# EvolEcolGroup/tidypopgen

Measured on AMD Instinct MI355X. Metric: SNP-genotypes/s (N x M) for IBS+KING+GRM+Fst+PCA; max |delta| vs CPU ref (cpu_baseline.parity), higher is better.
Workload: dtype fp4-e2m1 operands (exact integers, f32 accumulate) for the cross-products, the PCA Gram and the grouped counts, int8 (int32 accumulate) for the loadings, f64 for statistics

## Files before the change

include/tpg.h:

```cpp
#ifndef TPG_H
#define TPG_H

#include <stddef.h>
#include <stdint.h>

#ifdef __cplusplus
extern "C" {
#endif

#define TPG_OK 0
#define TPG_EINVAL 1
#define TPG_EHIP 2
#define TPG_EUNSUPPORTED 3
#define TPG_ENUMERIC 4

typedef struct tpg_ctx tpg_ctx;
typedef struct tpg_fbm tpg_fbm;
typedef struct tpg_view tpg_view;
typedef struct tpg_pairwise tpg_pairwise;
typedef struct tpg_comm tpg_comm;
typedef struct tpg_multi tpg_multi;

const char* tpg_last_error(void);
const char* tpg_version(void);
// ... 391 lines not shown
  size_t bytes_up;
  size_t bytes_down;
  size_t budget_bytes;
  size_t planned_bytes;
  size_t state_bytes;
  size_t peak_device_bytes;
  double seconds;
  double seconds_first_sweep;
} tpg_stream_report;

int tpg_stream_run(tpg_ctx* ctx, tpg_stream* s, const tpg_stream_job* job, tpg_stream_report* report);
int tpg_multi_stream_run(tpg_multi* mg, tpg_stream* s, const tpg_stream_job* job, tpg_stream_report* report);

typedef struct tpg_stream_qc_job {
  size_t struct_size;
  const int32_t* rowInd1;
  int64_t n;
  const int32_t* colInd1;
  int64_t m;
  const double* code256;
  const int32_t* groupIds0;
  int ngroups;
  int midp;
  int32_t* loci_counts;
  double* hwe_p;
  int32_t* grouped_counts;
  double* grouped_hwe_p;
  int32_t* indiv_counts;
} tpg_stream_qc_job;
int tpg_stream_qc(tpg_ctx* ctx, tpg_stream* s, const tpg_stream_qc_job* job, tpg_stream_report* report);

int tpg_pca_center_scale(tpg_ctx* ctx, const tpg_view* v, double* center, double* scale);
int tpg_pca_gram(tpg_ctx* ctx, const tpg_view* v, const double* center, const double* scale, double* K);
int tpg_pca_gram_add(tpg_ctx* ctx, const tpg_view* v, const double* center, const double* scale, double* K);
int tpg_pca_partial_svd(tpg_ctx* ctx, const tpg_view* v, int k, double* d, double* u, double* vload,
                        double* center, double* scale, double* square_frobenius);
int tpg_pca_random_svd(tpg_ctx* ctx, const tpg_view* v, int k, double tol, double* d, double* u, double* vload,
                       double* center, double* scale, double* square_frobenius);
int tpg_sym_eig_topk(tpg_ctx* ctx, const double* K, int64_t n, int k, double* lambda, double* U);
int tpg_pca_loadings(tpg_ctx* ctx, const tpg_view* v, const double* center, const double* scale,
                     const double* U, const double* d, int k, double* vload);
int tpg_fbm256_prod_and_rowSumsSq(tpg_ctx* ctx, const tpg_view* v, const double* center,
                                  const double* scale, const double* V, int K, double* XV, double* rss);
int tpg_square_frobenius(tpg_ctx* ctx, const tpg_view* v, const double* center, const double* scale,
                         double* out);
int tpg_fbm256_valid_prod(tpg_ctx* ctx, const tpg_view* v, const double* Tab, int K, double* out);

#define TPG_PCA_OP_TOL_FLOOR 1e-8
int tpg_pca_zt_prod(tpg_ctx* ctx, const tpg_view* v, const double* center, const double* scale, const double* Q, int b,
                    double* W);
int tpg_pca_z_prod(tpg_ctx* ctx, const tpg_view* v, const double* center, const double* scale, const double* W, int b,
                   double* Y);
int tpg_pca_random_svd_op(tpg_ctx* ctx, const tpg_view* v, int k, double tol, double* d, double* u, double* vload,
                          double* center, double* scale, double* square_frobenius, int* n_apply);
size_t tpg_pca_op_scratch_bytes(int64_t n, int64_t m, int k);
int tpg_pca_gram_route_fits(tpg_ctx* ctx, int64_t n, int k, int* fits);

#define TPG_PCADAPT_MAX_K 64
#define TPG_SELECT_TILE 1024
int64_t tpg_select_tile(void);
int tpg_col_median_mad(tpg_ctx* ctx, const double* X, int64_t rows, int ncols, int64_t ld, double* med, double* mad,
                       int64_t* n_finite);
int tpg_pcadapt_zscores(tpg_ctx* ctx, const tpg_view* v, const double* U, int K, double* z, int64_t* n_valid);
int tpg_robust_dist_ogk(tpg_ctx* ctx, const double* Z, int64_t m, int K, double* dist, double* center, double* cov,
                        double* basis, int64_t* n_valid);
int tpg_pchisq_log10_upper(tpg_ctx* ctx, const double* x, int64_t count, int df, double* out);
// ... 84 lines not shown
```

tidypopgen_amd/_lib.py:

```python
from __future__ import annotations

import ctypes as C
import os

_HERE = os.path.dirname(os.path.abspath(__file__))
LIB_PATH = os.environ.get("TPG_LIB_PATH") or os.path.join(_HERE, "libtpg_hip.so")


class TpgError(RuntimeError):
    def __init__(self, code: int, msg: str):
        super().__init__(f"[tpg error {code}] {msg}")
        self.code = code


def build(force: bool = False) -> str:
    import subprocess

    csrc = os.path.join(_HERE, "csrc")
    cmd = ["make", "-C", csrc, "-j8", "-s"]
    if force:
        cmd.append("-B")
    subprocess.check_call(cmd)
    return LIB_PATH

# ... 206 lines not shown
    "tpg_comm_rank": (ci, [vp]),
    "tpg_comm_size": (ci, [vp]),
    "tpg_shard_loci": (ci, [i64, ci, ci, vp, vp]),
    "tpg_comm_allreduce_f64": (ci, [vp, vp, vp, i64]),
    "tpg_pairwise_buffer_bytes_sharded": (sz, [i64, ci]),
    "tpg_pairwise_create_sharded": (ci, [vp, vp, i64, vp]),
    "tpg_pairwise_reduce": (ci, [vp, vp, vp]),
    "tpg_pairwise_reduce_begin": (ci, [vp, vp, vp]),
    "tpg_pairwise_reduce_end": (ci, [vp, vp, vp]),
    "tpg_pairwise_band": (ci, [vp, vp, vp]),
    "tpg_pairwise_band_of": (ci, [i64, ci, ci, vp, vp]),
    "tpg_pairwise_epilogues_sharded": (ci, [vp, vp, vp, ci, i64, vp, vp, vp, vp]),
    "tpg_pca_partial_svd_sharded": (ci, [vp, vp, vp, ci, vp, vp, vp, vp, vp, vp]),
    "tpg_multi_create": (ci, [ci, vp, vp]),
    "tpg_multi_destroy": (None, [vp]),
    "tpg_multi_ndev": (ci, [vp]),
    "tpg_multi_ctx": (vp, [vp, ci]),
    "tpg_multi_comm": (vp, [vp, ci]),
    "tpg_multi_pairwise": (ci, [vp, vp, i64, i64, vp, i64, vp, i64, ci, vp, vp, vp, vp]),
    "tpg_multi_grouped_alt_freq": (ci, [vp, vp, i64, i64, vp, i64, vp, i64, vp, vp, ci, vp, ci, vp]),
    "tpg_multi_pop_fst": (ci, [vp, vp, i64, i64, vp, i64, vp, i64, vp, vp, ci, vp, ci, vp, ci, ci, ci, vp, vp, vp]),
    "tpg_multi_pca_partial_svd": (ci, [vp, vp, i64, i64, vp, i64, vp, i64, vp, ci, vp, vp, vp, vp, vp, vp]),
    "tpg_stream_open_host": (ci, [vp, vp, i64, i64, sz, vp]),
    "tpg_stream_open_bk": (ci, [vp, cstr, i64, i64, sz, vp]),
    "tpg_stream_open_bed": (ci, [vp, cstr, i64, i64, sz, vp]),
    "tpg_stream_open_bed_host": (ci, [vp, vp, i64, i64, sz, vp]),
    "tpg_stream_open_synth": (ci, [vp, u64, i64, i64, ci, u32, ci, sz, vp]),
    "tpg_stream_close": (None, [vp]),
    "tpg_stream_run": (ci, [vp, vp, P(StreamJob), P(StreamReport)]),
    "tpg_multi_stream_run": (ci, [vp, vp, P(StreamJob), P(StreamReport)]),
    "tpg_stream_qc": (ci, [vp, vp, P(StreamQcJob), P(StreamReport)]),
    "tpg_pca_center_scale": (ci, [vp, vp, vp, vp]),
    "tpg_pca_gram": (ci, [vp, vp, vp, vp, vp]),
    "tpg_pca_gram_add": (ci, [vp, vp, vp, vp, vp]),
    "tpg_pca_partial_svd": (ci, [vp, vp, ci, vp, vp, vp, vp, vp, vp]),
    "tpg_pca_random_svd": (ci, [vp, vp, ci, f64, vp, vp, vp, vp, vp, vp]),
    "tpg_sym_eig_topk": (ci, [vp, vp, i64, ci, vp, vp]),
    "tpg_pca_loadings": (ci, [vp, vp, vp, vp, vp, vp, ci, vp]),
    "tpg_fbm256_prod_and_rowSumsSq": (ci, [vp, vp, vp, vp, vp, ci, vp, vp]),
    "tpg_square_frobenius": (ci, [vp, vp, vp, vp, vp]),
    "tpg_fbm256_valid_prod": (ci, [vp, vp, vp, ci, vp]),
    "tpg_pca_zt_prod": (ci, [vp, vp, vp, vp, vp, ci, vp]),
    "tpg_pca_z_prod": (ci, [vp, vp, vp, vp, vp, ci, vp]),
    "tpg_pca_random_svd_op": (ci, [vp, vp, ci, f64, vp, vp, vp, vp, vp, vp, vp]),
    "tpg_pca_op_scratch_bytes": (sz, [i64, i64, ci]),
    "tpg_pca_gram_route_fits": (ci, [vp, i64, ci, vp]),
    "tpg_select_tile": (i64, []),
    "tpg_col_median_mad": (ci, [vp, vp, i64, ci, i64, vp, vp, vp]),
    "tpg_pcadapt_zscores": (ci, [vp, vp, vp, ci, vp, vp]),
    "tpg_robust_dist_ogk": (ci, [vp, vp, i64, ci, vp, vp, vp, vp, vp]),
    "tpg_pchisq_log10_upper": (ci, [vp, vp, i64, ci, vp]),
    "tpg_qchisq_median": (ci, [ci, vp]),
    "tpg_pcadapt": (ci, [vp, vp, vp, ci, vp, vp, vp, vp, vp, vp]),
    "tpg_view_select_loci": (ci, [vp, vp, vp, i64, vp]),
    "tpg_qnorm_upper": (ci, [f64, vp]),
    "tpg_rollmean_weights": (ci, [ci, vp]),
    "tpg_rollmean_segments": (ci, [vp, vp, i64, vp, i64, ci, vp]),
    "tpg_medcouple": (ci, [vp, vp, i64, vp]),
    "tpg_tukey_mc_up": (ci, [vp, vp, i64, f64, vp]),
    "tpg_pca_auto_svd": (ci, [vp, vp, vp, vp, ci, f64, ci, f64, i64, ci, vp]),
    "tpg_autosvd_count": (i64, [vp]),
    "tpg_autosvd_iters": (ci, [vp]),
    "tpg_autosvd_converged": (ci, [vp]),
    "tpg_autosvd_fetch": (ci, [vp, vp, vp, vp, vp, vp, vp, vp]),
    "tpg_autosvd_history": (ci, [vp, ci, vp, vp, vp]),
    "tpg_autosvd_outliers": (ci, [vp, ci, vp, vp]),
# ... 40 lines not shown
```

tidypopgen_amd/api.py:

```python
from __future__ import annotations

import ctypes as C
import math
from typing import Optional

import numpy as np

from . import _lib
from ._lib import check, lib

CODE_012 = np.full(256, np.nan)
CODE_012[:3] = [0.0, 1.0, 2.0]
CODE_IMPUTE_PRED = np.full(256, np.nan)
CODE_IMPUTE_PRED[:3] = [0.0, 1.0, 2.0]
CODE_IMPUTE_PRED[4:7] = [0.0, 1.0, 2.0]

FST_METHODS = {"Hudson": 0, "Nei87": 1, "WC84": 2}
IMPUTE_METHODS = {"mode": 1, "mean0": 2, "random": 3}


def _impute_method(method) -> int:
    if method not in IMPUTE_METHODS:
        raise ValueError(f"impute method must be one of {sorted(IMPUTE_METHODS)}, not {method!r}")
    return IMPUTE_METHODS[method]
# ... 2271 lines not shown
    check(lib.tpg_pairwise_fst_loop(ctx.h, FST_METHODS[method], _ptr(pairs_c), P, m,
                                    G, _ptr(n), *[_ptr(x) for x in mats], int(by_locus),
                                    int(return_num_dem), _ptr(tot), _ptr(a), _ptr(b)))
    return _fst_result(tot, a, b, by_locus or return_num_dem, return_num_dem)


def pairwise_fst_hudson_loop(pairwise_combn, n, freq_alt, freq_ref, by_locus=False, return_num_dem=False, ctx=None):
    return _fst_loop("Hudson", pairwise_combn, n, freq_alt, freq_ref, None, by_locus, return_num_dem, ctx)


def pairwise_fst_wc84_loop(pairwise_combn, n, freq_alt, het_obs, by_locus=False, return_num_dem=False, ctx=None):
    return _fst_loop("WC84", pairwise_combn, n, freq_alt, None, het_obs, by_locus, return_num_dem, ctx)


def pairwise_fst_nei87_loop(pairwise_combn, n, het_obs, freq_alt, freq_ref, by_locus=False, return_num_dem=False,
                            ctx=None):
    return _fst_loop("Nei87", pairwise_combn, n, freq_alt, freq_ref, het_obs, by_locus, return_num_dem, ctx)



def pca_center_scale(v: View):
    center, scale = np.zeros(v.m), np.zeros(v.m)
    check(lib.tpg_pca_center_scale(v.ctx.h, v.h, _ptr(center), _ptr(scale)))
    return center, scale


def pca_gram(v: View, center, scale) -> np.ndarray:
    K = np.zeros((v.n, v.n), order="F")
    center, scale = _f64(center), _f64(scale)
    check(lib.tpg_pca_gram(v.ctx.h, v.h, _ptr(center), _ptr(scale), _ptr(K)))
    return K


def sym_eig_topk(K, k: int, ctx: Optional[Context] = None):
    ctx = ctx or default_context()
    K = np.asfortranarray(K, dtype=float)
    n = K.shape[0]
    lam, U = np.zeros(k), np.zeros((n, k), order="F")
    check(lib.tpg_sym_eig_topk(ctx.h, _ptr(K), n, k, _ptr(lam), _ptr(U)))
    return lam, U


def pca_loadings(v: View, center, scale, U, d) -> np.ndarray:
    center, scale, d = _f64(center), _f64(scale), _f64(d)
    U = np.asfortranarray(U, dtype=float)
    k = U.shape[1]
    out = np.zeros((v.m, k), order="F")
    check(lib.tpg_pca_loadings(v.ctx.h, v.h, _ptr(center), _ptr(scale), _ptr(U), _ptr(d), k, _ptr(out)))
    return out


def _pca_view(X: FBM, ind_row, ind_col, code256, impute, impute_seed) -> View:
    if impute is None:
        return View(X, ind_row, ind_col, code256=code256)
    return View(X, ind_row, ind_col, code256=CODE_012).impute(impute, impute_seed)


def gt_pca_partialSVD(X: FBM, ind_row=None, ind_col=None, k: int = 10, total_var: bool = True,
                      code256=CODE_IMPUTE_PRED, impute: Optional[str] = None, impute_seed: int = 0) -> dict:
    v = _pca_view(X, ind_row, ind_col, code256, impute, impute_seed)
    d = np.zeros(k)
    u = np.zeros((v.n, k), order="F")
    vl = np.zeros((v.m, k), order="F")
    center, scale = np.zeros(v.m), np.zeros(v.m)
    fro = C.c_double()
    check(lib.tpg_pca_partial_svd(v.ctx.h, v.h, k, _ptr(d), _ptr(u), _ptr(vl), _ptr(center), _ptr(scale),
# ... 817 lines not shown
```

tidypopgen_amd/csrc/gramcls.hip:

```cpp
#include <math.h>
#include <string.h>

#include <algorithm>
#include <vector>

#include <hipcub/hipcub.hpp>

#include "common.h"
#include "devfrag.h"
#include "host/host_bits2.h"

constexpr int GA = 2, GB = 2, GP = GA * GB;
#define GCLS_SLAB (GP * 16 * 64)
#define GCLS_MAX_RUN 65536

__global__ void tpg_gcls_keys_kernel(const double* __restrict__ w, int64_t m, unsigned long long* __restrict__ key,
                                     uint32_t* __restrict__ idx) {
  for (int64_t j = blockIdx.x * (int64_t)blockDim.x + threadIdx.x; j < m; j += (int64_t)gridDim.x * blockDim.x) {
    const unsigned long long b = (unsigned long long)__double_as_longlong(w[j]);
    key[j] = (b + 16ull) & ~31ull;
    idx[j] = (uint32_t)j;
  }
}

// ... 37 lines not shown
__global__ void tpg_gcls_block_table_kernel(const unsigned long long* __restrict__ ukeys, const uint32_t* __restrict__ blk_start,
                                            const uint32_t* __restrict__ nblk, int nr, int64_t nblocks,
                                            unsigned long long* __restrict__ wblk) {
  for (int64_t b = blockIdx.x * (int64_t)blockDim.x + threadIdx.x; b < nblocks; b += (int64_t)gridDim.x * blockDim.x) {
    const int r = tpg_gcls_find_run(blk_start, nr, (uint32_t)b);
    const uint32_t o = (uint32_t)b - blk_start[r];
    const unsigned long long fl = (o + 1 == nblk[r] || (o % GCLS_MAX_RUN) == GCLS_MAX_RUN - 1) ? 1ull : 0ull;
    wblk[b] = ukeys[r] | fl;
  }
}

#define GCLS_GQ 6
#define GCLS_GMAX 64
#define GCLS_GRUN 16384
__global__ void tpg_gcls_block_table2_kernel(const unsigned long long* __restrict__ ukeys, const uint32_t* __restrict__ blk_start,
                                             const uint32_t* __restrict__ nblk, int nr, int64_t nblocks, int gmax, int gq,
                                             ulonglong2* __restrict__ wblk) {
  if (blockIdx.x == 0 && threadIdx.x < 4) wblk[nblocks + threadIdx.x] = make_ulonglong2(ukeys[nr - 1], 0ull);
  for (int64_t b = blockIdx.x * (int64_t)blockDim.x + threadIdx.x; b < nblocks; b += (int64_t)gridDim.x * blockDim.x) {
    const int r = tpg_gcls_find_run(blk_start, nr, (uint32_t)b);
    const uint32_t o = (uint32_t)b - blk_start[r];
    const bool class_end = o + 1 == nblk[r];
    bool full = (o % GCLS_GRUN) == GCLS_GRUN - 1;
    if (class_end)
      full = full || r == nr - 1 || (ukeys[r] >> (52 - gq)) != (ukeys[r + 1] >> (52 - gq)) ||
             (r % gmax) == gmax - 1 || blk_start[r] / GCLS_GRUN != (blk_start[r] + nblk[r]) / GCLS_GRUN;
    ulonglong2 e;
    e.x = ukeys[r] | (full ? 2ull : class_end ? 1ull : 0ull);
    e.y = 0;
    if (class_end && !full)
      e.y = (unsigned long long)__float_as_uint(
          (float)(__longlong_as_double((long long)ukeys[r]) - __longlong_as_double((long long)ukeys[r + 1])));
    wblk[b] = e;
  }
}

struct GclsSrc {
  const uint4* base;
  int sh;
  int64_t sa;
  int msk;
  int64_t sb, sq, sh1;
};

#define GSH_ROW 68
#define GSH_HS 140
#define GSH_WORDS (4 * 2 * GSH_HS)
template <bool CEN, int QW>
__global__ __launch_bounds__(256) void tpg_gcls_gather_kernel(GclsSrc S, int64_t Q,
                                                               const int32_t* __restrict__ src, int64_t nblocks,
                                                               int64_t rs2, uint4* __restrict__ T2g) {
  __shared__ __attribute__((aligned(16))) uint32_t shm[4][GSH_WORDS];
  const int lane = threadIdx.x & 63, wv = threadIdx.x >> 6;
  uint32_t* sh = shm[wv];
  const int g = lane & 3, x = lane >> 2, t_s = x & 3, t_hs = (x >> 2) & 1, t_hb = x >> 3;
  const uint4* rd_src = (const uint4*)(sh + x * GSH_ROW + 16 * g);
  uint32_t* wr_dst = sh + t_s * (2 * GSH_HS) + t_hs * GSH_HS + (g >> 1) * 4 + 2 * t_hb + (g & 1);
  const int r = lane & 31, ho = lane >> 5;
  const uint4* rd_dst = (const uint4*)(sh + (r >> 4) * GSH_HS + (r & 15) * 8 + ho * 4);
  const uint32_t uQ = (uint32_t)((Q + QW - 1) / QW), ntask = uQ * (uint32_t)rs2, step = gridDim.x * 4u;
  auto load_j = [&](uint32_t task, int32_t (&j)[2]) {
    j[0] = j[1] = -1;
    if (task < ntask) {
      const int64_t bp = task / uQ;
#pragma unroll
      for (int hb = 0; hb < 2; hb++)
// ... 419 lines not shown
    __builtin_amdgcn_fence(__ATOMIC_ACQUIRE, "workgroup");
    const int a = lane & 31, h = lane >> 5;
#pragma unroll 4
    for (int it = 0; it < 16; it++) {
      const int c = 2 * it + h;
      const int i1 = 32 * ti + a, k1 = 32 * tk + c;
      if (i1 < n && k1 < n) K[i1 + (int64_t)k1 * n] = tile[p][a][c];
      const int i2 = 32 * ti + c, k2 = 32 * tk + a;
      if (i2 < n && k2 < n) K[k2 + (int64_t)i2 * n] = tile[p][c][a];
    }
    __builtin_amdgcn_wave_barrier();
  }
}

static bool gcls_fold64(int64_t nruns, int64_t nblocks) {
  if (tpg_env_set("TPG_GRAM_FOLD64")) return tpg_env_int("TPG_GRAM_FOLD64", 0) != 0;
  return (double)nruns < 0.15 * (double)nblocks;
}

static double gcls_cost_classes(int64_t nunits, int64_t nruns, int64_t nblocks, int nwaves, int* bestS) {
  double best = -1;
  const bool f64 = gcls_fold64(nruns, nblocks);
  const double t_class = f64 ? 0.136 : GCLS2_T_CLASS, t_block = f64 ? 0.079 : GCLS2_T_BLOCK;
  for (int S = 2; S <= 32; S += 2) {
    if (nblocks / S < 4 && S > 2) break;
    const int64_t rounds = ceil_div(nunits * S, (int64_t)nwaves);
    const double per = ((double)nruns / S + 1.0) * GP * t_class + (double)ceil_div(nblocks, (int64_t)S) * GP * t_block + 6.0;
    const double cost = (double)rounds * per + (double)S * (double)nunits * 8.5e-3;
    if (best < 0 || cost < best * 0.995) { best = cost; *bestS = S; }
  }
  return best;
}

static int gram_classes_core(tpg_ctx* ctx, int64_t n, int64_t Q, int64_t m, const GclsSrc& src, const double* d_w, double* d_what,
                             double* d_K, bool force, bool* done, bool centred_ok) {
  *done = false;
  if (m >= (1ll << 31) - 64 || (tpg_env_set("TPG_GRAM_DIGITS") && !force)) return TPG_OK;
  DevArena B;
  unsigned long long *d_key = nullptr, *d_key2 = nullptr, *d_ukeys = nullptr;
  uint32_t *d_idx = nullptr, *d_idx2 = nullptr, *d_counts = nullptr, *d_cnt = nullptr, *d_nblk = nullptr, *d_estart = nullptr,
           *d_bstart = nullptr;
  int* d_nruns = nullptr;
  long long* d_totals = nullptr;
  void* d_tmp = nullptr;
  TPG_TRY(B.get(&d_key, (size_t)m)); TPG_TRY(B.get(&d_key2, (size_t)m)); TPG_TRY(B.get(&d_ukeys, (size_t)m));
  TPG_TRY(B.get(&d_idx, (size_t)m)); TPG_TRY(B.get(&d_idx2, (size_t)m)); TPG_TRY(B.get(&d_counts, (size_t)m));
  TPG_TRY(B.get(&d_cnt, (size_t)m)); TPG_TRY(B.get(&d_nblk, (size_t)m)); TPG_TRY(B.get(&d_estart, (size_t)m));
  TPG_TRY(B.get(&d_bstart, (size_t)m)); TPG_TRY(B.get(&d_nruns, 1)); TPG_TRY(B.get(&d_totals, 2));
  size_t t_sort = 0, t_rle = 0, t_scan = 0;
  TPG_HIP(hipcub::DeviceRadixSort::SortPairs(nullptr, t_sort, d_key, d_key2, d_idx, d_idx2, (int)m, 0, 64, ctx->stream));
  TPG_HIP(hipcub::DeviceRunLengthEncode::Encode(nullptr, t_rle, d_key2, d_ukeys, d_counts, d_nruns, (int)m, ctx->stream));
  TPG_HIP(hipcub::DeviceScan::ExclusiveSum(nullptr, t_scan, d_cnt, d_estart, (int)m, ctx->stream));
  const size_t t_bytes = std::max(t_sort, std::max(t_rle, t_scan));
  TPG_TRY(B.get((uint8_t**)&d_tmp, t_bytes));
  long long totals[2] = {0, 0};
  {
    ProfScope ps(ctx, "gcls_classes");
    hipLaunchKernelGGL(tpg_gcls_keys_kernel, dim3(1024), dim3(256), 0, ctx->stream, d_w, m, d_key, d_idx);
    size_t t = t_bytes;
    TPG_HIP(hipcub::DeviceRadixSort::SortPairs(d_tmp, t, d_key, d_key2, d_idx, d_idx2, (int)m, 0, 64, ctx->stream));
    t = t_bytes;
    TPG_HIP(hipcub::DeviceRunLengthEncode::Encode(d_tmp, t, d_key2, d_ukeys, d_counts, d_nruns, (int)m, ctx->stream));
    hipLaunchKernelGGL(tpg_gcls_run_blocks_kernel, dim3(1024), dim3(256), 0, ctx->stream, (const uint32_t*)d_counts,
                       (const int*)d_nruns, m, d_cnt, d_nblk);
    t = t_bytes;
    TPG_HIP(hipcub::DeviceScan::ExclusiveSum(d_tmp, t, d_cnt, d_estart, (int)m, ctx->stream));
    t = t_bytes;
    TPG_HIP(hipcub::DeviceScan::ExclusiveSum(d_tmp, t, d_nblk, d_bstart, (int)m, ctx->stream));
    hipLaunchKernelGGL(tpg_gcls_totals_kernel, dim3(1), dim3(1), 0, ctx->stream, (const int*)d_nruns,
                       (const uint32_t*)d_bstart, (const uint32_t*)d_nblk, d_totals);
  }
  TPG_HIP(tpg_fetch_small(ctx, totals, d_totals, sizeof(totals)));
  const int64_t nruns = totals[0], nblocks = totals[1];
  TPG_REQUIRE(nruns > 0 && nblocks > 0, TPG_EHIP, "class table is empty");

  const int nrtv = (int)ceil_div(n, 32);
  const int nI = (int)ceil_div(nrtv, GA), nJ = (int)ceil_div(nrtv, GB);
  std::vector<int2> order;
  const int PJ = 8;
  for (int pj = 0; pj * PJ < nJ; pj++) {
    const int j1 = std::min(nJ, pj * PJ + PJ);
    for (int I = 0; I < nI; I++)
      for (int J = pj * PJ; J < j1; J++)
        if (GB * J + GB - 1 >= GA * I) order.push_back(make_int2(I, J));
  }
  const int64_t nun = (int64_t)order.size();
  int ncu8 = ctx->num_cu / 8 * 8;
  if (ncu8 < 8) ncu8 = 8;
  const bool f64 = gcls_fold64(nruns, nblocks);
  static const bool no_cen = tpg_env_int("TPG_GRAM_CENTER", 1) == 0;
  const bool cen = centred_ok && !no_cen && !f64;
  const int nblk_grid = 2 * ncu8;
  const int nwaves = 4 * nblk_grid;
  int S = 2;
  const double cost_cls = gcls_cost_classes(nun, nruns, nblocks, nwaves, &S) + 350.0 + 1.25e-3 * (double)m * ((double)n / 5000.0);
  const int64_t nun_dig = (int64_t)nrtv * ceil_div((int64_t)nrtv, 4) / 2 + nrtv;
  const int t_dig = std::max(4, ((int)ceil(log2(2.0 * (double)n + 1.0)) + ctx->pca_digit_fbits + 7) / 7);
  const double cost_dig = (double)ceil_div(nun_dig, (int64_t)(4 * ncu8)) * ((double)ceil_div(m, 128) * 0.25 * t_dig) + 65.0;
  while ((nblocks / 2 + S) / S + 2 >= (1 << 21)) S += 2;
  if (tpg_env_set("TPG_DEBUG"))
    fprintf(stderr, "[tpg] gram classes: %lld classes, %lld blocks for %lld loci, S = %d, model %.0f us (digits %.0f us)\n",
            (long long)nruns, (long long)nblocks, (long long)m, S, cost_cls, cost_dig);
  if (cost_cls > cost_dig && !force && !tpg_env_set("TPG_GRAM_CLASSES")) return TPG_OK;

  int32_t* d_src = nullptr;
  double* d_slabs = nullptr;
  unsigned long long* d_wblk = nullptr;
  ulonglong2* d_wblk2 = nullptr;
  uint4* d_T2g = nullptr;
  int2* d_order = nullptr;
  TPG_TRY(B.get(&d_src, (size_t)nblocks * 64));
  if (f64) TPG_TRY(B.get(&d_wblk, (size_t)nblocks));
  else TPG_TRY(B.get(&d_wblk2, (size_t)nblocks + 4));
  const int64_t rs2 = (nblocks + 1) / 2;
  TPG_TRY(B.get(&d_T2g, (size_t)(4 * Q) * (size_t)rs2 * 64));
  TPG_TRY(B.get(&d_order, (size_t)nun));
  TPG_TRY(B.get(&d_slabs, (size_t)S * (size_t)nun * GCLS_SLAB));
  TPG_HIP(tpg_h2d_async(ctx, d_order, order.data(), sizeof(int2) * (size_t)nun));
  TPG_HIP(hipMemsetAsync(d_src, 0xFF, sizeof(int32_t) * (size_t)nblocks * 64, ctx->stream));
  {
    ProfScope ps(ctx, "gcls_layout");
    hipLaunchKernelGGL(tpg_gcls_place_kernel, dim3(1024), dim3(256), 0, ctx->stream, (const uint32_t*)d_idx2,
                       (const unsigned long long*)d_ukeys, (const uint32_t*)d_estart, (const uint32_t*)d_bstart, (int)nruns, m,
                       d_src, d_what);
    if (f64)
      hipLaunchKernelGGL(tpg_gcls_block_table_kernel, dim3(256), dim3(256), 0, ctx->stream, (const unsigned long long*)d_ukeys,
                         (const uint32_t*)d_bstart, (const uint32_t*)d_nblk, (int)nruns, nblocks, d_wblk);
    else
      hipLaunchKernelGGL(tpg_gcls_block_table2_kernel, dim3(256), dim3(256), 0, ctx->stream, (const unsigned long long*)d_ukeys,
                         (const uint32_t*)d_bstart, (const uint32_t*)d_nblk, (int)nruns, nblocks, GCLS_GMAX, GCLS_GQ, d_wblk2);
  }
  {
    const int64_t tasks = Q * rs2;
    if (tasks >= ((int64_t)1 << 31)) return TPG_OK;
    const unsigned grid = (unsigned)std::min<int64_t>(ceil_div(tasks, 4), (int64_t)ctx->num_cu * 16);
    const int qw = tpg_env_int("TPG_GATHER_QW", Q >= 4 ? 4 : Q >= 2 ? 2 : 1);
#define GATHER_GO(C, W) TPG_LAUNCH(ctx, "gcls_gather", (tpg_gcls_gather_kernel<C, W>), dim3(grid), dim3(256), 0, src, Q, (const int32_t*)d_src, nblocks, rs2, d_T2g)
    if (cen) { if (qw == 4) GATHER_GO(true, 4); else if (qw == 2) GATHER_GO(true, 2); else GATHER_GO(true, 1); }
    else { if (qw == 4) GATHER_GO(false, 4); else if (qw == 2) GATHER_GO(false, 2); else GATHER_GO(false, 1); }
#undef GATHER_GO
  }
  if (f64)
    TPG_LAUNCH(ctx, "pca_gram_classes", tpg_gcls_gram_kernel, dim3((unsigned)nblk_grid), dim3(256), 0, (const uint4*)d_T2g, nblocks,
               rs2, nrtv, (const unsigned long long*)d_wblk, (const int2*)d_order, nun, S, d_slabs);
  else if (cen) {
    (void)hipFuncSetAttribute((const void*)tpg_gcls_gram2_kernel<true>, hipFuncAttributeMaxDynamicSharedMemorySize, GCLS2_LDS_BYTES);
    TPG_LAUNCH(ctx, "pca_gram_classes", tpg_gcls_gram2_kernel<true>, dim3((unsigned)nblk_grid), dim3(256), GCLS2_LDS_BYTES,
               (const uint4*)d_T2g, nblocks, rs2, nrtv, (const ulonglong2*)d_wblk2, (const int2*)d_order, nun, S, d_slabs);
  } else {
    (void)hipFuncSetAttribute((const void*)tpg_gcls_gram2_kernel<false>, hipFuncAttributeMaxDynamicSharedMemorySize, GCLS2_LDS_BYTES);
    TPG_LAUNCH(ctx, "pca_gram_classes", tpg_gcls_gram2_kernel<false>, dim3((unsigned)nblk_grid), dim3(256), GCLS2_LDS_BYTES,
               (const uint4*)d_T2g, nblocks, rs2, nrtv, (const ulonglong2*)d_wblk2, (const int2*)d_order, nun, S, d_slabs);
  }
  TPG_LAUNCH(ctx, "gcls_assemble", tpg_gcls_assemble_kernel, dim3((unsigned)std::min<int64_t>(nun, 4096)), dim3(256), 0,
             (const double*)d_slabs, (const int2*)d_order, nun, S, (int)n, d_K);
  TPG_CHECK_LAUNCH();
  *done = true;
  return TPG_OK;
}

__global__ __launch_bounds__(256) void tpg_gcls_l2lm_kernel(const uint4* __restrict__ L, int64_t Q, int64_t n_lt,
                                                            uint4* __restrict__ LM) {
  __shared__ uint4 sh[32][8];
  for (int64_t task = blockIdx.x; task < tpg_lm_tasks(n_lt, Q); task += gridDim.x) {
    TpgLmSide l, lm;
    tpg_lm_task(task, Q, (int)threadIdx.x, l, lm);
    if (l.on) sh[l.row][l.col] = L[l.piece];
    __syncthreads();
    if (lm.on) LM[lm.piece] = sh[lm.row][lm.col];
    __syncthreads();
  }
}

int tpg_gram_classes(tpg_ctx* ctx, const tpg_view* v, const double* d_w, double* d_what, double* d_K, bool* done,
                     bool centred_ok) {
  *done = false;
  if (tpg_env_set("TPG_GRAM_DIGITS")) return TPG_OK;
  const int64_t n_lt = 4 * v->KG;
  DevBuf d_LM;
  if (!v->LM) {
    TPG_TRY(tpg_view_need_L(ctx, v));
    TPG_TRY(d_LM.alloc_n<uint4>((size_t)n_lt * 32 * (size_t)v->Q * 2));
    TPG_LAUNCH(ctx, "gcls_l2lm", tpg_gcls_l2lm_kernel, dim3((unsigned)std::min<int64_t>(n_lt * ((v->Q + 3) / 4), (int64_t)ctx->num_cu * 32)),
               dim3(256), 0, (const uint4*)v->L, v->Q, n_lt, d_LM.as<uint4>());
  }
  const GclsSrc src{v->LM ? v->LM : d_LM.as<uint4>(), 0, 2 * v->Q, 0, 0, 2, 1};
  const int rc = gram_classes_core(ctx, v->n, v->Q, v->m, src, d_w, d_what, d_K, false, done, centred_ok);
  d_LM.free();
  return rc;
}

#define GCLX_REC_WORDS(Q) (4 * (Q) + 2)

__global__ void tpg_gclx_keys_kernel(const int32_t* __restrict__ counts, int64_t m, int n, int32_t* __restrict__ key,
                                     int32_t* __restrict__ hist) {
  for (int64_t j = blockIdx.x * (int64_t)blockDim.x + threadIdx.x; j < m; j += (int64_t)gridDim.x * blockDim.x) {
    const int c = counts[4 * j + 1] + 2 * counts[4 * j + 2];
    const int k = min(c, 2 * n - c);
    key[j] = k;
    atomicAdd(&hist[k], 1);
  }
}

__global__ void tpg_gclx_dest_kernel(const int32_t* __restrict__ key, int64_t m, const uint8_t* __restrict__ owner,
                                     uint32_t* __restrict__ dest, uint32_t* __restrict__ idx, int32_t* __restrict__ per_dest) {
  for (int64_t j = blockIdx.x * (int64_t)blockDim.x + threadIdx.x; j < m; j += (int64_t)gridDim.x * blockDim.x) {
    const uint32_t d = owner[key[j]];
    dest[j] = d;
    idx[j] = (uint32_t)j;
    atomicAdd(&per_dest[d], 1);
  }
}

__global__ __launch_bounds__(256) void tpg_gclx_pack_kernel(const uint4* __restrict__ L, int64_t Q, const uint32_t* __restrict__ order,
                                                            const double* __restrict__ scale, int64_t m,
                                                            uint4* __restrict__ rec) {
  const int lane = threadIdx.x & 63;
  const int64_t recq = 2 * Q + 1;
  for (int64_t i = (int64_t)blockIdx.x * 4 + (threadIdx.x >> 6); i < m; i += (int64_t)gridDim.x * 4) {
    const uint32_t j = order[i];
    const uint4* p = L + ((int64_t)(j >> 5) * Q) * 64 + (j & 31);
    for (int64_t t = lane; t < 2 * Q; t += 64) rec[i * recq + t] = p[(t >> 1) * 64 + (t & 1) * 32];
// ... 156 lines not shown
```

Before: 145.1 billion.

## Build Gram weight classes with a hash dedupe instead of a full radix sort

Replaces the sort-based grouping of SNP weights into classes with a GPU hash-table dedupe, a ranking of the distinct keys, per-chunk histograms with a column scan, and a block-local radix-sort placement. The goal is to avoid sorting all m weights when the number of distinct weights is small. If there are more distinct weights than the table holds, it falls back to the sort path. It also exposes the plan through a C and Python API for inspection. Exchange: more kernel launches and an O(nd^2) rank kernel.

```diff
diff --git a/include/tpg.h b/include/tpg.h
--- a/include/tpg.h
+++ b/include/tpg.h
@@ -447,6 +447,8 @@
 
 int tpg_pca_center_scale(tpg_ctx* ctx, const tpg_view* v, double* center, double* scale);
 int tpg_pca_gram(tpg_ctx* ctx, const tpg_view* v, const double* center, const double* scale, double* K);
+int tpg_gram_class_plan(tpg_ctx* ctx, const double* w, int64_t m, int64_t* nruns, int64_t* nblocks, int* sorted, int32_t* src,
+                        int64_t* ukeys, uint32_t* nblk, uint32_t* bstart, double* what, int64_t* wblk, int64_t* wblk2);
 int tpg_pca_gram_add(tpg_ctx* ctx, const tpg_view* v, const double* center, const double* scale, double* K);
 int tpg_pca_partial_svd(tpg_ctx* ctx, const tpg_view* v, int k, double* d, double* u, double* vload,
                         double* center, double* scale, double* square_frobenius);
diff --git a/tidypopgen_amd/_lib.py b/tidypopgen_amd/_lib.py
--- a/tidypopgen_amd/_lib.py
+++ b/tidypopgen_amd/_lib.py
@@ -262,6 +262,7 @@
     "tpg_stream_qc": (ci, [vp, vp, P(StreamQcJob), P(StreamReport)]),
     "tpg_pca_center_scale": (ci, [vp, vp, vp, vp]),
     "tpg_pca_gram": (ci, [vp, vp, vp, vp, vp]),
+    "tpg_gram_class_plan": (ci, [vp, vp, i64, vp, vp, vp, vp, vp, vp, vp, vp, vp, vp]),
     "tpg_pca_gram_add": (ci, [vp, vp, vp, vp, vp]),
     "tpg_pca_partial_svd": (ci, [vp, vp, ci, vp, vp, vp, vp, vp, vp]),
     "tpg_pca_random_svd": (ci, [vp, vp, ci, f64, vp, vp, vp, vp, vp, vp]),
diff --git a/tidypopgen_amd/api.py b/tidypopgen_amd/api.py
--- a/tidypopgen_amd/api.py
+++ b/tidypopgen_amd/api.py
@@ -2327,6 +2327,26 @@
     return K
 
 
+def gram_class_plan(w, ctx: Optional[Context] = None) -> dict:
+    ctx = ctx or default_context()
+    w = _f64(w)
+    m = len(w)
+    nruns, nblocks, by_sort = C.c_int64(0), C.c_int64(0), C.c_int(0)
+    none = _ptr(None)
+    check(lib.tpg_gram_class_plan(ctx.h, _ptr(w), m, C.byref(nruns), C.byref(nblocks), C.byref(by_sort),
+                                  none, none, none, none, none, none, none))
+    nr, nb = nruns.value, nblocks.value
+    src = np.zeros(64 * nb, dtype=np.int32)
+    ukeys, nblk, bstart = np.zeros(nr, dtype=np.uint64), np.zeros(nr, dtype=np.uint32), np.zeros(nr, dtype=np.uint32)
+    what, wblk, wblk2 = np.zeros(m), np.zeros(nb, dtype=np.uint64), np.zeros(2 * (nb + 4), dtype=np.uint64)
+    check(lib.tpg_gram_class_plan(ctx.h, _ptr(w), m, C.byref(nruns), C.byref(nblocks), C.byref(by_sort), _ptr(src),
+                                  _ptr(ukeys), _ptr(nblk), _ptr(bstart), _ptr(what), _ptr(wblk), _ptr(wblk2)))
+    if (nruns.value, nblocks.value) != (nr, nb):
+        raise RuntimeError("the class plan changed between two calls on the same weights")
+    return dict(nruns=nr, nblocks=nb, sorted=bool(by_sort.value), src=src, ukeys=ukeys, nblk=nblk, bstart=bstart, what=what,
+                wblk=wblk, wblk2=wblk2)
+
+
 def sym_eig_topk(K, k: int, ctx: Optional[Context] = None):
     ctx = ctx or default_context()
     K = np.asfortranarray(K, dtype=float)
diff --git a/tidypopgen_amd/csrc/gramcls.hip b/tidypopgen_amd/csrc/gramcls.hip
--- a/tidypopgen_amd/csrc/gramcls.hip
+++ b/tidypopgen_amd/csrc/gramcls.hip
@@ -93,6 +93,213 @@
       e.y = (unsigned long long)__float_as_uint(
           (float)(__longlong_as_double((long long)ukeys[r]) - __longlong_as_double((long long)ukeys[r + 1])));
     wblk[b] = e;
+  }
+}
+
+#define GCLS_PLAN_SLOTS (1 << 16)
+#define GCLS_PLAN_CHUNKS 256
+#define GCLS_TILE 4096
+#define GCLS_HIST 8192
+#define GCLS_HASH_MUL 0x9E3779B97F4A7C15ull
+#define GCLS_PLAN_SAMPLE 65536
+__global__ void tpg_gcls_dedupe_kernel(const double* __restrict__ w, int64_t m, int64_t stride, unsigned long long* tab, int lg,
+                                       uint32_t cap, uint32_t* st, unsigned long long* __restrict__ dkeys,
+                                       uint32_t* __restrict__ slot_pos, uint32_t* __restrict__ lslot) {
+  const uint32_t mask = (1u << lg) - 1u;
+  for (int64_t i = blockIdx.x * (int64_t)blockDim.x + threadIdx.x; i * stride < m; i += (int64_t)gridDim.x * blockDim.x) {
+    const int64_t j = i * stride;
+    const unsigned long long key = ((unsigned long long)__double_as_longlong(w[j]) + 16ull) & ~31ull;
+    const unsigned long long mine = key | 1ull;
+    uint32_t h = (uint32_t)(((key >> 5) * GCLS_HASH_MUL) >> (64 - lg));
+    for (uint32_t probes = 0;; probes++) {
+      if (probes > mask) { st[1] = 1u; break; }
+      unsigned long long cur = tab[h];
+      if (cur == 0ull) {
+        if (*(volatile uint32_t*)&st[1]) return;
+        cur = atomicCAS(&tab[h], 0ull, mine);
+        if (cur == 0ull) {
+          const unsigned long long won = __ballot(1);
+          const int lane = (int)__lane_id(), leader = __ffsll((long long)won) - 1;
+          uint32_t base = 0;
+          if (lane == leader) base = atomicAdd(&st[0], (uint32_t)__popcll(won));
+          base = (uint32_t)__shfl((int)base, leader);
+          const uint32_t pos = base + (uint32_t)__popcll(won & ((1ull << lane) - 1ull));
+          if (pos < cap) { dkeys[pos] = key; slot_pos[h] = pos; }
+          else st[1] = 1u;
+          break;
+        }
+      }
+      if (cur == mine) break;
+      h = (h + 1u) & mask;
+    }
+    if (lslot) lslot[j] = h;
+  }
+}
+
+__global__ __launch_bounds__(256) void tpg_gcls_rank_kernel(const uint32_t* __restrict__ st, uint32_t cap,
+                                                            const unsigned long long* __restrict__ dkeys, uint32_t* __restrict__ rank) {
+  __shared__ unsigned long long oth[256];
+  if (st[1]) return;
+  const uint32_t nd = min(st[0], cap);
+  const uint32_t T = (nd + 255u) / 256u;
+  for (uint32_t p = blockIdx.x; p < T * T; p += gridDim.x) {
+    const uint32_t i = (p / T) * 256u + threadIdx.x, o = (p % T) * 256u + threadIdx.x;
+    oth[threadIdx.x] = o < nd ? dkeys[o] : ~0ull;
+    const unsigned long long mine = i < nd ? dkeys[i] : 0ull;
+    __syncthreads();
+    uint32_t c = 0;
+#pragma unroll 16
+    for (int k = 0; k < 256; k++) c += oth[k] < mine ? 1u : 0u;
+    if (i < nd && c) atomicAdd(&rank[i], c);
+    __syncthreads();
+  }
+}
+
+__global__ __launch_bounds__(1024) void tpg_gcls_count_kernel(const uint32_t* __restrict__ st, uint32_t cap,
+                                                              const uint32_t* __restrict__ slot_pos,
+                                                              const uint32_t* __restrict__ rank, const double* __restrict__ w,
+                                                              int64_t m, int64_t chunk,
+                                                              uint32_t* __restrict__ lrank, uint32_t* __restrict__ tbl,
+                                                              double* __restrict__ what) {
+  __shared__ uint32_t hist[GCLS_HIST];
+  if (st[1]) return;
+  const uint32_t nd = min(st[0], cap);
+  const int64_t j0 = blockIdx.x * chunk, j1 = min(m, j0 + chunk);
+  for (uint32_t base = 0; base < nd; base += GCLS_HIST) {
+    for (int t = threadIdx.x; t < GCLS_HIST; t += 1024) hist[t] = 0u;
+    __syncthreads();
+    for (int64_t j = j0 + threadIdx.x; j < j1; j += 1024) {
+      uint32_t r;
+      if (base == 0) {
+        r = rank[slot_pos[lrank[j]]];
+        lrank[j] = r;
+        if (what) what[j] = __longlong_as_double((long long)(((unsigned long long)__double_as_longlong(w[j]) + 16ull) & ~31ull));
+      } else
+        r = lrank[j];
+      if (r - base < (uint32_t)GCLS_HIST) atomicAdd(&hist[r - base], 1u);
+    }
+    __syncthreads();
+    for (uint32_t t = threadIdx.x; t < (uint32_t)GCLS_HIST && base + t < nd; t += 1024)
+      tbl[(size_t)blockIdx.x * cap + base + t] = hist[t];
+    __syncthreads();
+  }
+}
+
+__global__ __launch_bounds__(256) void tpg_gcls_colscan_kernel(const uint32_t* __restrict__ st, uint32_t cap, int nch,
+                                                               uint32_t* __restrict__ tbl, uint32_t* __restrict__ cnt) {
+  __shared__ uint32_t seg[8][32];
+  if (st[1]) return;
+  const uint32_t nd = min(st[0], cap);
+  const int x = threadIdx.x & 31, y = threadIdx.x >> 5;
+  const int per = (nch + 7) / 8, c0 = min(nch, y * per), c1 = min(nch, c0 + per);
+  for (uint32_t r0 = blockIdx.x * 32u; r0 < nd; r0 += gridDim.x * 32u) {
+    const uint32_t r = r0 + x;
+    uint32_t s = 0;
+    if (r < nd)
+      for (int c = c0; c < c1; c++) s += tbl[(size_t)c * cap + r];
+    seg[y][x] = s;
+    __syncthreads();
+    uint32_t run = 0;
+    for (int yy = 0; yy < y; yy++) run += seg[yy][x];
+    if (r < nd) {
+      for (int c = c0; c < c1; c++) {
+        const uint32_t t = tbl[(size_t)c * cap + r];
+        tbl[(size_t)c * cap + r] = run;
+        run += t;
+      }
+      if (y == 7) cnt[r] = run;
+    }
+    __syncthreads();
+  }
+}
+
+__global__ __launch_bounds__(1024) void tpg_gcls_book_kernel(const uint32_t* __restrict__ st, uint32_t cap,
+                                                             const uint32_t* __restrict__ cnt,
+                                                             const unsigned long long* __restrict__ dkeys,
+                                                             const uint32_t* __restrict__ rank, unsigned long long* __restrict__ ukeys,
+                                                             uint32_t* __restrict__ nblk, uint32_t* __restrict__ bstart,
+                                                             long long* __restrict__ totals) {
+  __shared__ uint32_t part[1024];
+  if (st[1]) {
+    if (threadIdx.x == 0) { totals[0] = 0; totals[1] = 0; totals[2] = 1; }
+    return;
+  }
+  const uint32_t nd = min(st[0], cap);
+  for (uint32_t i = threadIdx.x; i < nd; i += 1024u) ukeys[rank[i]] = dkeys[i];
+  const uint32_t per = (nd + 1023u) / 1024u, r0 = min(nd, threadIdx.x * per), r1 = min(nd, r0 + per);
+  uint32_t s = 0;
+  for (uint32_t r = r0; r < r1; r++) s += (cnt[r] + 63u) / 64u;
+  part[threadIdx.x] = s;
+  __syncthreads();
+  for (int off = 1; off < 1024; off <<= 1) {
+    const uint32_t v = (int)threadIdx.x >= off ? part[threadIdx.x - off] : 0u;
+    __syncthreads();
+    part[threadIdx.x] += v;
+    __syncthreads();
+  }
+  uint32_t run = part[threadIdx.x] - s;
+  for (uint32_t r = r0; r < r1; r++) {
+    const uint32_t nb = (cnt[r] + 63u) / 64u;
+    nblk[r] = nb;
+    bstart[r] = run;
+    run += nb;
+  }
+  if (threadIdx.x == 1023) { totals[0] = nd; totals[1] = part[1023]; totals[2] = 0; }
+}
+
+__global__ __launch_bounds__(1024) void tpg_gcls_place_ranked_kernel(const uint32_t* __restrict__ lrank,
+                                                                     const uint32_t* __restrict__ bstart, uint32_t* __restrict__ tbl,
+                                                                     uint32_t cap, uint32_t nd, int64_t m, int64_t chunk,
+                                                                     int32_t* __restrict__ src) {
+  using Sort = hipcub::BlockRadixSort<uint32_t, 1024, 4>;
+  using Scan = hipcub::BlockScan<int, 1024>;
+  __shared__ union {
+    typename Sort::TempStorage sort;
+    typename Scan::TempStorage scan;
+  } tmp;
+  __shared__ uint32_t skey[GCLS_TILE + 1];
+  const int rb = 32 - __clz((int)nd);
+  uint32_t* row = tbl + (size_t)blockIdx.x * cap;
+  const int64_t j0 = blockIdx.x * chunk, j1 = min(m, j0 + chunk);
+  const bool more = chunk > GCLS_TILE;
+  for (int64_t t0 = j0; t0 < j1; t0 += GCLS_TILE) {
+    uint32_t k[4];
+#pragma unroll
+    for (int q = 0; q < 4; q++) {
+      const uint32_t l = threadIdx.x * 4u + q;
+      k[q] = ((t0 + l < j1 ? lrank[t0 + l] : nd) << 12) | l;
+    }
+    Sort(tmp.sort).Sort(k, 12, 12 + rb);
+#pragma unroll
+    for (int q = 0; q < 4; q++) skey[threadIdx.x * 4 + q] = k[q];
+    if (threadIdx.x == 0) skey[GCLS_TILE] = 0xFFFFFFFFu;
+    __syncthreads();
+    int head[4], last = 0;
+#pragma unroll
+    for (int q = 0; q < 4; q++) {
+      const int p = threadIdx.x * 4 + q;
+      if (p > 0 && (skey[p - 1] >> 12) != (k[q] >> 12)) last = p;
+      head[q] = last;
+    }
+    int before = 0;
+    Scan(tmp.scan).ExclusiveScan(last, before, 0, hipcub::Max());
+#pragma unroll
+    for (int q = 0; q < 4; q++) {
+      const uint32_t r = k[q] >> 12;
+      head[q] = max(head[q], before);
+      if (r < nd)
+        src[(int64_t)bstart[r] * 64 + row[r] + (uint32_t)((int)(threadIdx.x * 4 + q) - head[q])] = (int32_t)(t0 + (k[q] & 4095u));
+    }
+    __syncthreads();
+    if (more) {
+#pragma unroll
+      for (int q = 0; q < 4; q++) {
+        const int p = threadIdx.x * 4 + q;
+        const uint32_t r = k[q] >> 12;
+        if (r < nd && (skey[p + 1] >> 12) != r) row[r] += (uint32_t)(p - head[q] + 1);
+      }
+      __syncthreads();
+    }
   }
 }
 
@@ -578,11 +785,82 @@
   return best;
 }
 
-static int gram_classes_core(tpg_ctx* ctx, int64_t n, int64_t Q, int64_t m, const GclsSrc& src, const double* d_w, double* d_what,
-                             double* d_K, bool force, bool* done, bool centred_ok) {
-  *done = false;
-  if (m >= (1ll << 31) - 64 || (tpg_env_set("TPG_GRAM_DIGITS") && !force)) return TPG_OK;
-  DevArena B;
+struct GclsPlan {
+  unsigned long long* ukeys = nullptr;
+  uint32_t *nblk = nullptr, *bstart = nullptr;
+  int64_t nruns = 0, nblocks = 0;
+  bool sorted = false;
+  uint32_t *idx2 = nullptr, *estart = nullptr;
+  uint32_t *lrank = nullptr, *tbl = nullptr;
+  uint32_t cap = 0;
+  int nch = 0;
+  int64_t chunk = 0;
+};
+
+static int gcls_plan_lg_slots() {
+  const int want = std::min(std::max(tpg_env_int("TPG_GCLS_PLAN_SLOTS", GCLS_PLAN_SLOTS), 4), GCLS_PLAN_SLOTS);
+  int lg = 2;
+  while ((2 << lg) <= want) lg++;
+  return lg;
+}
+
+static int gcls_plan_sort(tpg_ctx* ctx, DevArena& B, const double* d_w, int64_t m, GclsPlan* P);
+
+static int gcls_plan_hash(tpg_ctx* ctx, DevArena& B, const double* d_w, int64_t m, double* d_what, GclsPlan* P, bool* overflow) {
+  const int lg = gcls_plan_lg_slots();
+  const size_t slots = (size_t)1 << lg;
+  const uint32_t cap = (uint32_t)(slots / 2);
+  const int64_t ntiles = ceil_div(m, (int64_t)GCLS_TILE);
+  P->chunk = ceil_div(ntiles, (int64_t)GCLS_PLAN_CHUNKS) * GCLS_TILE;
+  P->nch = (int)ceil_div(m, P->chunk);
+  P->cap = cap;
+  unsigned long long *d_tab = nullptr, *d_dkeys = nullptr;
+  uint32_t *d_slot_pos = nullptr, *d_cnt = nullptr;
+  long long* d_totals = nullptr;
+  TPG_TRY(B.get(&d_tab, slots + 2 + cap / 2)); TPG_TRY(B.get(&d_dkeys, (size_t)cap)); TPG_TRY(B.get(&d_slot_pos, slots));
+  TPG_TRY(B.get(&d_cnt, (size_t)cap)); TPG_TRY(B.get(&d_totals, 3));
+  TPG_TRY(B.get(&P->ukeys, (size_t)cap)); TPG_TRY(B.get(&P->nblk, (size_t)cap)); TPG_TRY(B.get(&P->bstart, (size_t)cap));
+  TPG_TRY(B.get(&P->lrank, (size_t)m)); TPG_TRY(B.get(&P->tbl, (size_t)P->nch * cap));
+  uint32_t *d_st = (uint32_t*)(d_tab + slots), *d_rank = d_st + 4;
+  long long totals[3] = {0, 0, 0};
+  {
+    ProfScope ps(ctx, "gcls_classes");
+    TPG_HIP(hipMemsetAsync(d_tab, 0, sizeof(unsigned long long) * (slots + 2 + cap / 2), ctx->stream));
+    if (m > 2 * GCLS_PLAN_SAMPLE)
+      hipLaunchKernelGGL(tpg_gcls_dedupe_kernel, dim3(GCLS_PLAN_SAMPLE / 256), dim3(256), 0, ctx->stream, d_w, m,
+                         m / GCLS_PLAN_SAMPLE, d_tab, lg, cap, d_st, d_dkeys, d_slot_pos, (uint32_t*)nullptr);
+    hipLaunchKernelGGL(tpg_gcls_dedupe_kernel, dim3((unsigned)std::min<int64_t>(ceil_div(m, (int64_t)256), 2048)), dim3(256), 0,
+                       ctx->stream, d_w, m, (int64_t)1, d_tab, lg, cap, d_st, d_dkeys, d_slot_pos, P->lrank);
+    hipLaunchKernelGGL(tpg_gcls_rank_kernel, dim3(1024), dim3(256), 0, ctx->stream, (const uint32_t*)d_st, cap,
+                       (const unsigned long long*)d_dkeys, d_rank);
+    hipLaunchKernelGGL(tpg_gcls_count_kernel, dim3((unsigned)P->nch), dim3(1024), 0, ctx->stream, (const uint32_t*)d_st, cap,
+                       (const uint32_t*)d_slot_pos, (const uint32_t*)d_rank, d_w, m, P->chunk, P->lrank, P->tbl, d_what);
+    hipLaunchKernelGGL(tpg_gcls_colscan_kernel, dim3(std::min<unsigned>(cap / 32 + 1, 1024)), dim3(256), 0, ctx->stream,
+                       (const uint32_t*)d_st, cap, P->nch, P->tbl, d_cnt);
+    hipLaunchKernelGGL(tpg_gcls_book_kernel, dim3(1), dim3(1024), 0, ctx->stream, (const uint32_t*)d_st, cap,
+                       (const uint32_t*)d_cnt, (const unsigned long long*)d_dkeys, (const uint32_t*)d_rank, P->ukeys, P->nblk,
+                       P->bstart, d_totals);
+  }
+  TPG_HIP(tpg_fetch_small(ctx, totals, d_totals, sizeof(totals)));
+  P->nruns = totals[0];
+  P->nblocks = totals[1];
+  *overflow = totals[2] != 0;
+  return TPG_OK;
+}
+
+static int gcls_plan_classes(tpg_ctx* ctx, DevArena& B, const double* d_w, int64_t m, double* d_what, GclsPlan* P) {
+  const char* e = getenv("TPG_GCLS_PLAN");
+  if (!(e && !strcmp(e, "sort"))) {
+    bool overflow = false;
+    TPG_TRY(gcls_plan_hash(ctx, B, d_w, m, d_what, P, &overflow));
+    if (!overflow) return TPG_OK;
+    if (tpg_env_set("TPG_DEBUG")) fprintf(stderr, "[tpg] gram classes: more than %u distinct weights, sorting\n", P->cap);
+    *P = GclsPlan();
+  }
+  return gcls_plan_sort(ctx, B, d_w, m, P);
+}
+
+static int gcls_plan_sort(tpg_ctx* ctx, DevArena& B, const double* d_w, int64_t m, GclsPlan* P) {
   unsigned long long *d_key = nullptr, *d_key2 = nullptr, *d_ukeys = nullptr;
   uint32_t *d_idx = nullptr, *d_idx2 = nullptr, *d_counts = nullptr, *d_cnt = nullptr, *d_nblk = nullptr, *d_estart = nullptr,
            *d_bstart = nullptr;
@@ -617,7 +895,42 @@
                        (const uint32_t*)d_bstart, (const uint32_t*)d_nblk, d_totals);
   }
   TPG_HIP(tpg_fetch_small(ctx, totals, d_totals, sizeof(totals)));
-  const int64_t nruns = totals[0], nblocks = totals[1];
+  P->ukeys = d_ukeys; P->nblk = d_nblk; P->bstart = d_bstart; P->idx2 = d_idx2; P->estart = d_estart;
+  P->nruns = totals[0];
+  P->nblocks = totals[1];
+  P->sorted = true;
+  return TPG_OK;
+}
+
+static int gcls_plan_place(tpg_ctx* ctx, const GclsPlan& P, int64_t m, int32_t* d_src, double* d_what) {
+  TPG_HIP(hipMemsetAsync(d_src, 0xFF, sizeof(int32_t) * (size_t)P.nblocks * 64, ctx->stream));
+  if (P.sorted)
+    hipLaunchKernelGGL(tpg_gcls_place_kernel, dim3(1024), dim3(256), 0, ctx->stream, (const uint32_t*)P.idx2,
+                       (const unsigned long long*)P.ukeys, (const uint32_t*)P.estart, (const uint32_t*)P.bstart, (int)P.nruns, m,
+                       d_src, d_what);
+  else
+    hipLaunchKernelGGL(tpg_gcls_place_ranked_kernel, dim3((unsigned)P.nch), dim3(1024), 0, ctx->stream, (const uint32_t*)P.lrank,
+                       (const uint32_t*)P.bstart, P.tbl, P.cap, (uint32_t)P.nruns, m, P.chunk, d_src);
+  return TPG_OK;
+}
+
+static void gcls_plan_tables(tpg_ctx* ctx, const GclsPlan& P, unsigned long long* d_wblk, ulonglong2* d_wblk2) {
+  if (d_wblk)
+    hipLaunchKernelGGL(tpg_gcls_block_table_kernel, dim3(256), dim3(256), 0, ctx->stream, (const unsigned long long*)P.ukeys,
+                       (const uint32_t*)P.bstart, (const uint32_t*)P.nblk, (int)P.nruns, P.nblocks, d_wblk);
+  else
+    hipLaunchKernelGGL(tpg_gcls_block_table2_kernel, dim3(256), dim3(256), 0, ctx->stream, (const unsigned long long*)P.ukeys,
+                       (const uint32_t*)P.bstart, (const uint32_t*)P.nblk, (int)P.nruns, P.nblocks, GCLS_GMAX, GCLS_GQ, d_wblk2);
+}
+
+static int gram_classes_core(tpg_ctx* ctx, int64_t n, int64_t Q, int64_t m, const GclsSrc& src, const double* d_w, double* d_what,
+                             double* d_K, bool force, bool* done, bool centred_ok) {
+  *done = false;
+  if (m >= (1ll << 31) - 64 || (tpg_env_set("TPG_GRAM_DIGITS") && !force)) return TPG_OK;
+  DevArena B;
+  GclsPlan P;
+  TPG_TRY(gcls_plan_classes(ctx, B, d_w, m, d_what, &P));
+  const int64_t nruns = P.nruns, nblocks = P.nblocks;
   TPG_REQUIRE(nruns > 0 && nblocks > 0, TPG_EHIP, "class table is empty");
 
   const int nrtv = (int)ceil_div(n, 32);
@@ -663,18 +976,10 @@
   TPG_TRY(B.get(&d_order, (size_t)nun));
   TPG_TRY(B.get(&d_slabs, (size_t)S * (size_t)nun * GCLS_SLAB));
   TPG_HIP(tpg_h2d_async(ctx, d_order, order.data(), sizeof(int2) * (size_t)nun));
-  TPG_HIP(hipMemsetAsync(d_src, 0xFF, sizeof(int32_t) * (size_t)nblocks * 64, ctx->stream));
   {
     ProfScope ps(ctx, "gcls_layout");
-    hipLaunchKernelGGL(tpg_gcls_place_kernel, dim3(1024), dim3(256), 0, ctx->stream, (const uint32_t*)d_idx2,
-                       (const unsigned long long*)d_ukeys, (const uint32_t*)d_estart, (const uint32_t*)d_bstart, (int)nruns, m,
-                       d_src, d_what);
-    if (f64)
-      hipLaunchKernelGGL(tpg_gcls_block_table_kernel, dim3(256), dim3(256), 0, ctx->stream, (const unsigned long long*)d_ukeys,
-                         (const uint32_t*)d_bstart, (const uint32_t*)d_nblk, (int)nruns, nblocks, d_wblk);
-    else
-      hipLaunchKernelGGL(tpg_gcls_block_table2_kernel, dim3(256), dim3(256), 0, ctx->stream, (const unsigned long long*)d_ukeys,
-                         (const uint32_t*)d_bstart, (const uint32_t*)d_nblk, (int)nruns, nblocks, GCLS_GMAX, GCLS_GQ, d_wblk2);
+    TPG_TRY(gcls_plan_place(ctx, P, m, d_src, d_what));
+    gcls_plan_tables(ctx, P, d_wblk, d_wblk2);
   }
   {
     const int64_t tasks = Q * rs2;
@@ -734,6 +1039,50 @@
   const int rc = gram_classes_core(ctx, v->n, v->Q, v->m, src, d_w, d_what, d_K, false, done, centred_ok);
   d_LM.free();
   return rc;
+}
+
+extern "C" int tpg_gram_class_plan(tpg_ctx* ctx, const double* w, int64_t m, int64_t* nruns, int64_t* nblocks, int* sorted,
+                                   int32_t* src, int64_t* ukeys, uint32_t* nblk, uint32_t* bstart, double* what, int64_t* wblk,
+                                   int64_t* wblk2) {
+  TpgEnter _enter(ctx);
+  TPG_REQUIRE(ctx && w && nruns && nblocks, TPG_EINVAL, "null argument");
+  TPG_REQUIRE(m > 0 && m < (1ll << 31) - 64, TPG_EINVAL, "bad m = %lld", (long long)m);
+  InBuf iw;
+  TPG_TRY(iw.init(ctx, w, sizeof(double) * (size_t)m));
+  DevArena B;
+  GclsPlan P;
+  double* d_what = nullptr;
+  TPG_TRY(B.get(&d_what, (size_t)m));
+  TPG_TRY(gcls_plan_classes(ctx, B, iw.dev<double>(), m, d_what, &P));
+  TPG_REQUIRE(P.nruns > 0 && P.nblocks > 0, TPG_EHIP, "class table is empty");
+  *nruns = P.nruns;
+  *nblocks = P.nblocks;
+  if (sorted) *sorted = P.sorted ? 1 : 0;
+  if (src || what) {
+    int32_t* d_src = nullptr;
+    TPG_TRY(B.get(&d_src, (size_t)P.nblocks * 64));
+    TPG_TRY(gcls_plan_place(ctx, P, m, d_src, d_what));
+    TPG_TRY(tpg_deliver(ctx, src, (const int32_t*)d_src, (size_t)P.nblocks * 64));
+    TPG_TRY(tpg_deliver(ctx, what, (const double*)d_what, (size_t)m));
+  }
+  if (wblk) {
+    unsigned long long* d_wblk = nullptr;
+    TPG_TRY(B.get(&d_wblk, (size_t)P.nblocks));
+    gcls_plan_tables(ctx, P, d_wblk, nullptr);
+    TPG_TRY(tpg_deliver(ctx, wblk, (const int64_t*)d_wblk, (size_t)P.nblocks));
+  }
+  if (wblk2) {
+    ulonglong2* d_wblk2 = nullptr;
+    TPG_TRY(B.get(&d_wblk2, (size_t)P.nblocks + 4));
+    gcls_plan_tables(ctx, P, nullptr, d_wblk2);
+    TPG_TRY(tpg_deliver(ctx, wblk2, (const int64_t*)d_wblk2, 2 * ((size_t)P.nblocks + 4)));
+  }
+  TPG_TRY(tpg_deliver(ctx, ukeys, (const int64_t*)P.ukeys, (size_t)P.nruns));
+  TPG_TRY(tpg_deliver(ctx, nblk, (const uint32_t*)P.nblk, (size_t)P.nruns));
+  TPG_TRY(tpg_deliver(ctx, bstart, (const uint32_t*)P.bstart, (size_t)P.nruns));
+  TPG_CHECK_LAUNCH();
+  TPG_HIP(hipStreamSynchronize(ctx->stream));
+  return TPG_OK;
 }
 
 #define GCLX_REC_WORDS(Q) (4 * (Q) + 2)
```

Result: no change. 146.1 billion, median of 6 (+0.7%).
